# marvinx97/cloud

Measured on AMD Instinct MI355X. Metric: images/sec ResNet-50 via run() at 1/2/4/8 MI355X; run()→first-step latency, higher is better.
Workload: dtype bf16

## Files before the change

cloud_amd/config.py:

```python
from __future__ import annotations

import os
from dataclasses import dataclass


@dataclass(frozen=True)
class Var:
    name: str
    type: type
    default: object
    doc: str
    area: str


_VARS = [
    Var("CLOUD_AMD_JOBS_DIR", str, "./jobs", "where run() stages job directories", "launcher"),
    Var("CLOUD_AMD_HOME", str, "~/.cloud_amd", "per-user state: the job-id index (jobs/<id> -> job directory) that "
        "python -m cloud_amd.jobs uses to find a job from any directory", "launcher"),
    Var("CLOUD_AMD_STAGE_COPY", bool, False, "stage code files by copying too (default: code "
        "hard-linked, every other file copied; a running job then never sees in-place edits of its sources)", "launcher"),
    Var("CLOUD_AMD_CPU_AFFINITY", bool, True, "launcher pins each GPU rank to the cores of its GPU's NUMA node "
        "(KFD io_links + sysfs cpulist), split between the ranks on that node; 0 = leave placement to the OS",
        "launcher"),
    Var("CLOUD_AMD_NUMA_ROOT", str, "/sys/devices/system/node", "sysfs NUMA-node tree read for rank CPU placement "
# ... 28 lines not shown
        "M, N >= 256), 'reg' (register staging); any other name selects 'auto'", "ops"),
    Var("CLOUD_AMD_WGRAD_BLOCKS", int, 512, "convolution weight gradients: split-K so that about this many "
        "workgroups run (tiles x splits); fewer splits = less fp32 slab traffic, more = fuller CUs", "ops"),
    Var("CLOUD_AMD_WGRAD_BLOCKS_SMALLM", int, 512, "convolution weight gradients with <= 128 output channels "
        "(ResNet stem, layers 1-2): split-K workgroup target", "ops"),
    Var("CLOUD_AMD_STEM_WGRAD_BLOCKS", int, 2048, "space-to-depth stem weight gradient (the last kernel of the "
        "backward pass): split-K workgroup target", "ops"),
    Var("CLOUD_AMD_DENSE_WGRAD_BLOCKS", int, 640, "dense-layer weight gradients (BERT): split-K workgroup target "
        "(round 4, same box: 640 -> 6,993 / 6,993 seq/s, 768 -> 6,962 / 6,952, 1024 -> 6,892 / 6,911, 512 -> "
        "6,865 / 6,896; profiles/r4_s36/)",
        "ops"),
    Var("CLOUD_AMD_DENSE_WGRAD_256", bool, False, "dense-layer weight gradients whose 256 x 256 tiles times a split "
        "count fill one round of the chip (BERT QKV / FFN) run on the two-phase 256 core with that split (measured "
        "3 % slower on BERT than the 128 core's 1024-workgroup split: 6,749 / 6,754 vs 6,952 / 6,940 seq/s)", "ops"),
    Var("CLOUD_AMD_TAPMASK", bool, True, "convolutions: tap-mask / incremental buffer-mode gather loaders; 0 keeps "
        "the general per-chunk decode loaders (A/B runs)", "ops"),
    Var("CLOUD_AMD_SPLIT_XCD", bool, True, "split-K GEMM/conv grids: give each XCD contiguous (split, tile) "
        "ranges so the tiles of one K chunk share an L2; 0 remaps tiles only (A/B runs)", "ops"),
    Var("CLOUD_AMD_BN_APPLY_BLOCKS", int, 0, "BatchNorm apply passes (fwd y/mask, bwd dz): total workgroups of "
        "the HBM stream; 0 = the reduction kernels' tiling", "ops"),
    Var("CLOUD_AMD_BN_APPLY_ILV", bool, True, "BatchNorm apply passes: 1 = RP-row groups dealt round-robin to "
        "the workgroups (one contiguous sweep); 0 = one contiguous row chunk per workgroup", "ops"),
    Var("CLOUD_AMD_CONV_TALL", bool, True, "<= 64-channel 3x3 convolutions (fwd, stride-1 dgrad): 256 x 64 tiles "
        "with 4 x 1 waves; 0 = 128 x 64 with 2 x 2 waves", "ops"),
    Var("CLOUD_AMD_STEM_LDS", bool, True, "space-to-depth stem convolution forward on the LDS-resident patch + filter "
        "kernel (csrc/include/ca_conv_stem.h); 0 = the implicit-GEMM row-segment loader", "ops"),
    Var("CLOUD_AMD_STEM_TALL", bool, True, "space-to-depth stem convolution on the tall 256 x 64 tiles too (0.88 -> "
        "0.72 ms per call at b1024); 0 = 128 x 64 tiles (A/B runs)", "ops"),
    Var("CLOUD_AMD_STEM_BWD_RECOMPUTE", bool, True, "ResNet stem tail backward: a statistics-only max-pool "
        "backward pass, then the BN-backward apply recomputes the pooled gradient per 2x2 block (the 112x112 "
        "gradient is never written: 3.3 GB fewer per step at b1024).  With the window loads issued ahead of "
        "any branch: 0.65 + 0.90 ms against 1.09 + 0.94 for write-then-apply, +0.8 % end to end "
        "(profiles/r4_s44/); 0 = write g and run the separate apply pass", "ops"),
    Var("CLOUD_AMD_BN_GROUPS_MAX", int, 512, "BatchNorm statistics: most groups of the first-level reduction of the "
        "per-tile partial rows (1..512; ~64 rows per group)", "ops"),
    Var("CLOUD_AMD_GEMM_LIB", str, "never", "plain bf16 GEMMs (bias / accumulate only, no fused epilogue): 'never' "
        "(default: every GEMM on the in-tree kernels, the same engine on every box and rank), 'auto' (diagnostic: "
        "times the in-tree kernel against hipBLASLt once per shape and keeps the faster), 'always' "
        "(ops/raw.py PlainGemmPolicy)", "ops"),
    Var("CLOUD_AMD_GEMM_PRW", bool, True, "forward 1x1 convolutions with N = 256, K = 64 (ResNet layer-1 conv3 "
        "and shortcut): persistent resident-weight core (csrc/include/ca_gemm_prw.h); 0 = the tiled 128 core",
        "ops"),
    Var("CLOUD_AMD_GEMM_PRWN", bool, True, "forward 1x1 convolutions N = 512 / K = 128 and N = 1024 / K = 256 with "
        "BN statistics (ResNet stage-2 / stage-3 conv3): the persistent core with the weight resident in column "
        "chunks (ca_gemm_prw.h); 0 = the tiled 128 core", "ops"),
    Var("CLOUD_AMD_SMALLK_SET", str, "", "bench/smallk_gemm.py shape set ('conv3': the conv3 expansions of "
        "stages 2-4)", "bench"),
    Var("CLOUD_AMD_EPI_PF", bool, True, "GEMM epilogues that read memory or run an activation (BN-statistics "
        "forward 1x1 convs, BERT bias/GELU/GELU'/beta dense layers): 4 staged output rows in flight per trip", "ops"),
    Var("CLOUD_AMD_ATTN_FUSED_BWD", bool, True, "attention at S = 64 / 128: one workgroup per (batch, head) for "
        "the forward and a single fused backward kernel; 0 keeps the 64-query-block kernels", "ops"),
    Var("CLOUD_AMD_CONV_HALO_WGRAD", bool, True, "the weight gradient of the same 3x3 / 64-channel / width-56 "
        "convolutions on the LDS-resident kernel (ca_conv_halo.h conv3x3_halo_wgrad: 64 x 576 partial in registers, "
        "one fp32 slab per workgroup); 0 = implicit GEMM (A/B)", "ops"),
    Var("CLOUD_AMD_LN_BWD16", bool, False, "LayerNorm backward on 16-wave blocks, one row per wave, the block's "
        "partials summed by a fixed LDS tree (measured 2.8 % slower on BERT beside the weight-gradient side stream; "
        "default: 4-wave blocks walking four rows per wave)", "ops"),
    Var("CLOUD_AMD_GEMM_256X96", bool, True, "forward GEMMs whose 256 x 96 grid fills whole rounds while the 128 x "
        "128 grid leaves a partial one (BERT QKV, M = 8192, N = 2304) run on 256 x 96 tiles; 0 = off (A/B)", "ops"),
    Var("CLOUD_AMD_BN_FIN_RPG", int, 512, "BatchNorm statistics finalize: partial rows per group block (64-512)", "ops"),
    Var("CLOUD_AMD_BN_FIN_MERGED", bool, True, "BatchNorm statistics from many partial rows: group reduction and "
        "per-channel finalize in ONE launch (last block per 64 channels finalizes, agent-scope ticket); 0 = two "
        "launches (A/B runs)", "ops"),
    Var("CLOUD_AMD_CONV_HALO", int, 1, "3x3 / stride-1 / 64-channel convolutions at width 56 (ResNet-50 "
        "stage 1) forward and input gradient on the LDS-resident kernel (ca_conv_halo.h: input patch and all 9 taps "
        "in LDS, persistent grid); 0 = implicit-GEMM tiles, 2 = halo kernel without the software-pipelined "
# ... 198 lines not shown
```

cloud_amd/models/resnet.py:

```python
from __future__ import annotations

import torch
import torch.nn as nn

from . import fused_block
from .. import config
from ..ops import conv as conv_ops
from ..ops import pooling as pool_ops
from .layers import BatchNormAct, Conv2d, GlobalAvgPool, Linear, MaxPool2d


class Bottleneck(nn.Module):
    expansion = 4

    def __init__(self, cin, width, stride=1, dtype=torch.bfloat16, device=None, zero_init_residual=True):
        super().__init__()
        cout = width * self.expansion
        self.conv1 = Conv2d(cin, width, 1, dtype=dtype, device=device)
        self.bn1 = BatchNormAct(width, relu=True, device=device)
        self.conv2 = Conv2d(width, width, 3, stride=stride, padding=1, dtype=dtype, device=device)
        self.bn2 = BatchNormAct(width, relu=True, device=device)
        self.conv3 = Conv2d(width, cout, 1, dtype=dtype, device=device)
        self.bn3 = BatchNormAct(cout, relu=True, zero_init=zero_init_residual, device=device)
        self.fused_stats = True
        self.fused_block = True
        self.downsample = None
        if stride != 1 or cin != cout:
            self.downsample = nn.ModuleDict({
                "conv": Conv2d(cin, cout, 1, stride=stride, dtype=dtype, device=device),
                "bn": BatchNormAct(cout, relu=False, device=device),
            })

    def forward(self, x, next_block=None):
        if self.fused_block and fused_block.can_fuse(self, x):
            return fused_block.bottleneck_forward(self, x, next_block)
        fused_block.check_not_pending(x)
        identity = x
        fs = self.fused_stats
        if self.downsample is not None:
            identity = self.downsample["bn"](self.downsample["conv"](x, stats=fs))
        out = self.bn1(self.conv1(x, stats=fs))
        out = self.bn2(self.conv2(out, stats=fs))
        return self.bn3(self.conv3(out, stats=fs), residual=identity)


class ResNet(nn.Module):
    def __init__(self, layers=(3, 4, 6, 3), num_classes=1000, in_channels=3, stem_channels_pad=0,
                 dtype=torch.bfloat16, device=None, zero_init_residual=True):
        super().__init__()
        self.in_channels = in_channels
        self.stem_cin = in_channels + stem_channels_pad
        self.conv1 = Conv2d(self.stem_cin, 64, 7, stride=2, padding=3, dtype=dtype, device=device)
        self.bn1 = BatchNormAct(64, relu=True, device=device)
        self.maxpool = MaxPool2d(3, 2, 1)
        self.stem_s2d = True
        blocks = []
        cin = 64
        for i, (n, width) in enumerate(zip(layers, (64, 128, 256, 512))):
            for j in range(n):
                stride = 2 if (j == 0 and i > 0) else 1
                blocks.append(Bottleneck(cin, width, stride, dtype=dtype, device=device,
                                         zero_init_residual=zero_init_residual))
                cin = width * Bottleneck.expansion
        self.layers = nn.Sequential(*blocks)
        self.pool = GlobalAvgPool()
        self.fc = Linear(cin, num_classes, dtype=dtype, device=device)

    def forward(self, x):
        c1 = self.conv1
        if self.stem_s2d and x.shape[-1] == self.in_channels and conv_ops.stem_s2d_ok(x, c1.weight, c1.stride,
                                                                                         c1.padding):
            x = self._stem_tail(conv_ops.stem_conv_s2d(x, c1.weight, stats=True))
        else:
            if self.stem_cin != self.in_channels:
                x = torch.nn.functional.pad(x, (0, self.stem_cin - self.in_channels))
            x = self._stem_tail(self.conv1(x, stats=True))
        if self.layers._forward_hooks or self.layers._forward_pre_hooks:
            x = self.layers(x)
        else:
            blocks = list(self.layers)
            for i, blk in enumerate(blocks):
                x = blk(x, blocks[i + 1] if i + 1 < len(blocks) else None)
        return self.fc(self.pool(x))

    def _stem_tail(self, out):
        z, part = out if isinstance(out, tuple) else (out, None)
        if config.get("CLOUD_AMD_STEM_TAIL") and pool_ops.stem_tail_ok(z, self.bn1, self.maxpool, part):
            return pool_ops.stem_bn_relu_maxpool(z, self.bn1, part)
        return self.maxpool(self.bn1((z, part) if part is not None else z))


def resnet50(**kw):
    kw.setdefault("stem_channels_pad", 5)
    return ResNet((3, 4, 6, 3), **kw)


def resnet18_like_small(**kw):
    return ResNet((1, 1, 1, 1), **kw)
```

cloud_amd/ops/conv.py:

```python
from __future__ import annotations

import os

import torch
import torch.nn.functional as F

from .. import config
from . import _ext, gemm, raw


def _out(n, k, s, p):
    return (n + 2 * p - k) // s + 1


def _conv_mode():
    return os.environ.get("CLOUD_AMD_CONV", "native")


def _native_conv_ok(x, w):
    Cin = x.shape[-1]
    Cout = w.shape[0]
    return (x.dtype == torch.bfloat16 and w.dtype == torch.bfloat16 and Cin % 8 == 0 and Cout % 8 == 0
            and x.is_contiguous() and x.numel() < 2 ** 31)

# ... 70 lines not shown
    Cout = g.shape[0]
    return g.view(Cout, 4, 4, 2, 2, 4).permute(0, 1, 3, 2, 4, 5).reshape(Cout, 8, 8, 4)[:, :7, :7, :cx]


class _StemS2DFn(torch.autograd.Function):

    @staticmethod
    def forward(ctx, x, w, param, stats):
        ext = _ext.load(required=True)
        N, H, W, cx = x.shape
        Cout = w.shape[0]
        OH, OW = _out(H, 7, 2, 3), _out(W, 7, 2, 3)
        Hs, Ws = OH + 3, OW + 3
        st = _ext.stream_handle(x.device)
        xs = torch.empty((N, Hs, Ws, 16), dtype=torch.bfloat16, device=x.device)
        ext.stem_s2d(x.data_ptr(), xs.data_ptr(), N, H, W, cx, Hs, Ws, 3, st)
        ws = _s2d_weight(w, cx)
        y = torch.empty((N, OH, OW, Cout), dtype=torch.bfloat16, device=x.device)
        ext.conv_fwd(xs.data_ptr(), ws.data_ptr(), y.data_ptr(), N, Hs, Ws, 16, Cout, 4, 4, 1, 1, 0, 0,
                     _ext.ptr(stats), st)
        ctx.save_for_backward(xs)
        ctx.param, ctx.cx, ctx.wshape = param, cx, w.shape
        return y

    @staticmethod
    def backward(ctx, dy):
        from . import raw

        (xs,) = ctx.saved_tensors
        dy = dy.contiguous()
        Cout = dy.shape[-1]
        g = torch.zeros((Cout, 4, 4, 16), dtype=torch.float32, device=dy.device)
        raw.conv_wgrad(dy, xs, g.shape, 1, 0, out=g, beta=0.0, blocks=config.get("CLOUD_AMD_STEM_WGRAD_BLOCKS"))
        gw = _s2d_weight_grad(g, ctx.cx)
        param = ctx.param
        sink = gemm._grad_sink(param) if param is not None else None
        if sink is not None:
            sink[..., :ctx.cx] += gw.to(sink.dtype)
            from ..parallel import ddp

            ddp.notify_grad_ready(param)
            return None, None, None, None
        full = torch.zeros(ctx.wshape, dtype=torch.float32, device=dy.device)
        full[..., :ctx.cx] = gw
        if param is not None:
            return None, None, full.to(param.dtype), None
        return None, full.to(torch.bfloat16), None, None


def stem_s2d_ok(x, w, stride, padding):
    return (_conv_mode() == "native" and x.is_cuda and x.dtype == torch.bfloat16 and w.dtype == torch.bfloat16
            and tuple(w.shape[1:3]) == (7, 7) and stride == 2 and padding == 3 and x.shape[-1] <= 4
            and x.shape[-1] <= w.shape[-1] and x.is_contiguous() and not x.requires_grad and _ext.use_native(x, w))


def stem_conv_s2d(x, w, stats=False):
    N, H, W, _ = x.shape
    Cout = w.shape[0]
    OH, OW = _out(H, 7, 2, 3), _out(W, 7, 2, 3)
    part = None
    if stats:
        rows = _ext.load(required=True).conv_stat_rows(N, OH + 3, OW + 3, 16, Cout, 4, 4, 1, 1, 0, 0)
        part = torch.empty((rows, 2, Cout), dtype=torch.float32, device=x.device)
    param = w if (w.is_leaf and w.requires_grad) else None
    y = _StemS2DFn.apply(x, w.detach() if param is not None else w, param, part)
    return (y, part) if stats else y


def stats_buffer(rows, channels, device):
    return torch.empty(((rows + 127) // 128, 2, channels), dtype=torch.float32, device=device)


def conv2d_nhwc(x, w, bias=None, stride=1, padding=0, stats=False):
    N, H, W, Cin = x.shape
    Cout, KH, KW, Cin_w = w.shape
    assert Cin == Cin_w, f"channel mismatch {Cin} vs {Cin_w}"
    native = _conv_mode() == "native" and x.is_cuda and _native_conv_ok(x, w) and _ext.use_native(x, w)
    part = None
    if KH == 1 and KW == 1 and padding == 0 and stride == 1:
        x2 = x.reshape(N * H * W, Cin)
# ... 21 lines not shown
```

csrc/bindings.cpp:

```cpp
#include <atomic>
#include <mutex>
#include <hip/hip_runtime.h>
#include <pybind11/pybind11.h>
#include <pybind11/stl.h>
#include <stdint.h>

#include <stdexcept>
#include <string>
#include <vector>

namespace py = pybind11;
typedef uint16_t bf16_t;

extern "C" {
int ca_sgd_step(float*, void*, int, float*, bf16_t*, const float*, const float*, long, int, int, hipStream_t);
int ca_adam_step(float*, void*, int, float*, float*, bf16_t*, const float*, const float*, long, int, int, hipStream_t);
int ca_rmsprop_step(float*, void*, int, float*, float*, bf16_t*, const float*, const float*, long, int, hipStream_t);
int ca_sumsq(const void*, int, long, float*, hipStream_t);
int ca_scale(void*, int, long, const float*, hipStream_t);
long ca_bn_workspace_floats(long, int);
int ca_bn_fwd(const bf16_t*, const bf16_t*, bf16_t*, long, int, const float*, const float*, float, float,
              float*, float*, float*, float*, float*, float*, int, uint8_t*, hipStream_t);
int ca_bn_apply(const bf16_t*, const bf16_t*, bf16_t*, long, int, const float*, int, hipStream_t);
int ca_bn_fwd_partials(const bf16_t*, const bf16_t*, bf16_t*, long, int, const float*, int, const float*, const float*,
// ... 21 lines not shown
                           hipStream_t);
int ca_gemm_xa_dw(const bf16_t*, const bf16_t*, const uint8_t*, const float*, const float*, const float*, long,
                  const bf16_t*, long, bf16_t*, long, int, int, int, float, const bf16_t*, const uint8_t*,
                  const bf16_t*, const uint8_t*, float*, const bf16_t*, float*, const bf16_t*, long, void*, int, float,
                  float*, int, hipStream_t);
int ca_dgrad_gemm(int, const bf16_t*, long, const bf16_t*, long, bf16_t*, long, int, int, int, float, const bf16_t*,
                  const uint8_t*, const bf16_t*, const uint8_t*, float*, hipStream_t, const bf16_t*, float*, int, int,
                  int);
int ca_conv_dgrad_bnstats(const bf16_t*, const bf16_t*, bf16_t*, int, int, int, int, int, int, int, int, int, int,
                          int, float, const bf16_t*, const uint8_t*, float*, hipStream_t);
int ca_u8_normalize(const uint8_t*, bf16_t*, long, int, const float*, const float*, hipStream_t);
int ca_stem_s2d(const bf16_t*, bf16_t*, int, int, int, int, int, int, int, hipStream_t);
int ca_softmax_xent(const void*, int, const int64_t*, int, int, float, float, float*, float*, void*, hipStream_t);
int ca_softmax_xent_batch(const void*, long, int, const int64_t*, int, int, float, float, float*, float*, void*, float*,
                          float,
                          hipStream_t);
int ca_maxpool_fwd(const bf16_t*, bf16_t*, uint8_t*, int, int, int, int, int, int, int, int, int, hipStream_t);
int ca_maxpool_bwd(const bf16_t*, const uint8_t*, bf16_t*, int, int, int, int, int, int, int, int, int, hipStream_t);
int ca_gap_fwd(const bf16_t*, void*, int, int, int, int, hipStream_t);
int ca_gap_bwd(const void*, int, bf16_t*, int, int, int, hipStream_t);
int ca_gmp_fwd(const bf16_t*, bf16_t*, float*, int, int, int, hipStream_t);
int ca_gmp_bwd(const void*, int, const bf16_t*, const bf16_t*, const float*, bf16_t*, int, int, int, hipStream_t);
int ca_gemm_bf16(int, const bf16_t*, long, const bf16_t*, long, bf16_t*, long, int, int, int, float*, float,
                 hipStream_t);
int ca_gemm_set_core(int);
int ca_gemm_set_xa_n256(int);
int ca_gemm_stat_rows(int, int, int, long, long, long);
int ca_bn_relu_maxpool_s2k3(const bf16_t*, const float*, bf16_t*, uint8_t*, int, int, int, int, int, int, hipStream_t);
int ca_maxpool_bnstats_parts(int, int, int, int);
int ca_maxpool_bwd_s2k3_bnstats(const bf16_t*, const bf16_t*, const uint8_t*, const bf16_t*, bf16_t*, float*, int, int,
                                int, int, int, int, hipStream_t);
int ca_maxpool_bwd_s2k3_bnapply(const bf16_t*, const bf16_t*, const uint8_t*, const bf16_t*, const float*, bf16_t*, int,
                                int, int, int, int, int, hipStream_t);
int ca_conv_fwd_ex(const bf16_t*, const bf16_t*, bf16_t*, int, int, int, int, int, int, int, int, int, int, int,
                   const float*, int, hipStream_t);
int ca_conv_fwd(const bf16_t*, const bf16_t*, bf16_t*, int, int, int, int, int, int, int, int, int, int, int, float*,
                hipStream_t);
int ca_conv_dgrad(const bf16_t*, const bf16_t*, bf16_t*, int, int, int, int, int, int, int, int, int, int, int, float,
                  hipStream_t, int);
int ca_conv_wgrad(const bf16_t*, const bf16_t*, void*, int, float, int, int, int, int, int, int, int, int, int, int,
                  int, int, float*, hipStream_t);
int ca_splitk_reduce(const float*, int, long, void*, int, float, hipStream_t);
int ca_grad_finalize_multi(const uint64_t*, const float*, int, hipStream_t);
int ca_cls_head_max_labels();
int ca_cls_head_fwd(const bf16_t*, long, const float*, const float*, float*, int, int, int, float, uint64_t,
                    hipStream_t);
int ca_cls_head_bwd(const float*, const bf16_t*, long, const float*, bf16_t*, float*, float*, int, int, int, float,
                    uint64_t, hipStream_t);
int ca_gemm_splitk(int, const bf16_t*, long, const bf16_t*, long, void*, int, float, int, int, int, int, float*,
                   hipStream_t);
int ca_gemm_splitk_effective(int, int);
int ca_gemm_ex(int, const bf16_t*, long, const bf16_t*, long, bf16_t*, long, int, int, int, float*, float, const float*,
               int, bf16_t*, const bf16_t*, long, hipStream_t);
long ca_ln_workspace_floats(long, int);
int ca_ln_fwd(const bf16_t*, const bf16_t*, const float*, const float*, bf16_t*, bf16_t*, float*, float*, long, int,
              float, float, uint64_t, float, uint64_t, const float*, hipStream_t);
int ca_ln_bwd(const bf16_t*, const bf16_t*, const float*, const float*, const float*, bf16_t*, bf16_t*, float*, float*,
              int, float*, long, int, float, uint64_t, float, uint64_t, hipStream_t, float*);
long ca_colsum_workspace_floats(long, int);
int ca_colsum(const bf16_t*, long, int, long, float*, int, float*, hipStream_t);
int ca_act_grad(const bf16_t*, long, int, const bf16_t*, bf16_t*, long, int, int, hipStream_t);
int ca_pad_cols(const void*, long, int, void*, int, long, long, int, hipStream_t);
int ca_slice_acc(const float*, long, void*, int, long, int, hipStream_t);
int ca_pad_cols_multi(const long*, int, hipStream_t);
int ca_splitk_bias_act(const float*, int, long, int, const float*, int, bf16_t*, hipStream_t);
int ca_embed_sum(const int32_t*, const int32_t*, const float*, const float*, const float*, bf16_t*, long, int, int, int,
// ... 221 lines not shown
  m.def("gemm_bf16", [](int layout, u64 A, long lda, u64 B, long ldb, u64 C, long ldc, int M, int N, int K,
                        u64 stats, float beta, u64 s) {
    check(ca_gemm_bf16(layout, P(const bf16_t*, A), lda, P(const bf16_t*, B), ldb, P(bf16_t*, C), ldc, M, N, K,
                       P(float*, stats), beta, S(s)), "gemm_bf16");
  });
  m.def("conv_fwd", [](u64 x, u64 w, u64 y, int Nb, int H, int W, int Cin, int Cout, int KH, int KW, int sh, int sw,
                       int ph, int pw, u64 stats, u64 s) {
    check(ca_conv_fwd(P(const bf16_t*, x), P(const bf16_t*, w), P(bf16_t*, y), Nb, H, W, Cin, Cout, KH, KW, sh, sw, ph,
                      pw, P(float*, stats), S(s)), "conv_fwd");
  });
  m.def("bn_relu_maxpool_s2k3", [](u64 z, u64 ss, u64 y, u64 idx, int N, int H, int W, int C, int OH, int OW,
                                   u64 s) {
    check(ca_bn_relu_maxpool_s2k3(P(const bf16_t*, z), P(const float*, ss), P(bf16_t*, y), P(uint8_t*, idx), N, H, W,
                                  C, OH, OW, S(s)), "bn_relu_maxpool_s2k3");
  });
  m.def("gemm_set_core", [](int kind) { return ca_gemm_set_core(kind); });
  m.def("gemm_set_xa_n256", [](int mode) { return ca_gemm_set_xa_n256(mode); });
  m.def("experimental_built", []() { return false; });
  m.def("gemm_set_streamk", [](int) { return -1; });
  m.def("maxpool_bnstats_parts", [](int N, int H, int W, int C) { return ca_maxpool_bnstats_parts(N, H, W, C); });
  m.def("maxpool_bwd_s2k3_bnstats", [](u64 dy, u64 yp, u64 idx, u64 z, u64 g, u64 part, int N, int H, int W, int C,
                                       int OH, int OW, u64 s) {
    check(ca_maxpool_bwd_s2k3_bnstats(P(const bf16_t*, dy), P(const bf16_t*, yp), P(const uint8_t*, idx),
                                      P(const bf16_t*, z), P(bf16_t*, g), P(float*, part), N, H, W, C, OH, OW, S(s)),
          "maxpool_bwd_s2k3_bnstats");
  });
  m.def("maxpool_bwd_s2k3_bnapply", [](u64 dy, u64 yp, u64 idx, u64 z, u64 coef, u64 dz, int N, int H, int W, int C,
                                       int OH, int OW, u64 s) {
    check(ca_maxpool_bwd_s2k3_bnapply(P(const bf16_t*, dy), P(const bf16_t*, yp), P(const uint8_t*, idx),
                                      P(const bf16_t*, z), P(const float*, coef), P(bf16_t*, dz), N, H, W, C, OH, OW,
                                      S(s)),
          "maxpool_bwd_s2k3_bnapply");
  });
  m.def("conv_fwd_ex", [](u64 x, u64 w, u64 y, int Nb, int H, int W, int Cin, int Cout, int KH, int KW, int sh,
                          int sw, int ph, int pw, u64 bias, int act, u64 s) {
    check(ca_conv_fwd_ex(P(const bf16_t*, x), P(const bf16_t*, w), P(bf16_t*, y), Nb, H, W, Cin, Cout, KH, KW, sh, sw,
                         ph, pw, P(const float*, bias), act, S(s)), "conv_fwd_ex");
  });
  m.def("conv_dgrad", [](u64 dy, u64 w, u64 dx, int Nb, int H, int W, int Cin, int Cout, int KH, int KW, int sh,
                         int sw, int ph, int pw, float beta, u64 s, int skip_empty) {
    check(ca_conv_dgrad(P(const bf16_t*, dy), P(const bf16_t*, w), P(bf16_t*, dx), Nb, H, W, Cin, Cout, KH, KW, sh, sw,
                        ph, pw, beta, S(s), skip_empty), "conv_dgrad");
  }, py::arg("dy"), py::arg("w"), py::arg("dx"), py::arg("Nb"), py::arg("H"), py::arg("W"), py::arg("Cin"),
        py::arg("Cout"), py::arg("KH"), py::arg("KW"), py::arg("sh"), py::arg("sw"), py::arg("ph"), py::arg("pw"),
        py::arg("beta"), py::arg("s"), py::arg("skip_empty") = 0);
  m.def("conv_wgrad", [](u64 dy, u64 x, u64 dw, int dw_bf16, float beta, int Nb, int H, int W, int Cin, int Cout,
                         int KH, int KW, int sh, int sw, int ph, int pw, int splits, u64 ws, u64 s) {
    check(ca_conv_wgrad(P(const bf16_t*, dy), P(const bf16_t*, x), P(void*, dw), dw_bf16, beta, Nb, H, W, Cin, Cout,
                        KH, KW, sh, sw, ph, pw, splits, P(float*, ws), S(s)), "conv_wgrad");
  });
  m.def("grad_finalize_multi", [](const std::vector<uint64_t>& jobs, const std::vector<float>& betas, u64 s) {
    const int n = (int)betas.size();
    if ((long)jobs.size() != 12L * n) throw std::runtime_error("grad_finalize_multi: 12 fields per job");
    check(ca_grad_finalize_multi(jobs.data(), betas.data(), n, S(s)), "grad_finalize_multi");
  });
  m.def("cls_head_max_labels", []() { return ca_cls_head_max_labels(); });
  m.def("cls_head_fwd", [](u64 pooled, long ldp, u64 wc, u64 bc, u64 logits, int B, int C, int L, float p, u64 seed,
                           u64 s) {
    check(ca_cls_head_fwd(P(const bf16_t*, pooled), ldp, P(const float*, wc), P(const float*, bc), P(float*, logits),
                          B, C, L, p, seed, S(s)), "cls_head_fwd");
  });
  m.def("cls_head_bwd", [](u64 dl, u64 pooled, long ldp, u64 wc, u64 dpre, u64 gwc, u64 gbc, int B, int C, int L,
                           float p, u64 seed, u64 s) {
    check(ca_cls_head_bwd(P(const float*, dl), P(const bf16_t*, pooled), ldp, P(const float*, wc), P(bf16_t*, dpre),
                          P(float*, gwc), P(float*, gbc), B, C, L, p, seed, S(s)), "cls_head_bwd");
  });
// ... 96 lines not shown
```

csrc/kernels/pool.hip:

```cpp
#include "ca_common.h"

namespace {

__global__ void __launch_bounds__(256) maxpool_fwd_kernel(const bf16_t* __restrict__ x, bf16_t* __restrict__ y,
                                                         uint8_t* __restrict__ idx, int N, int H, int W, int C,
                                                         int OH, int OW, int k, int s, int p) {
  const int CT = C / 8;
  const long total = (long)N * OH * OW * CT;
  for (long t = (long)blockIdx.x * blockDim.x + threadIdx.x; t < total; t += (long)gridDim.x * blockDim.x) {
    const int vc = (int)(t % CT);
    long r = t / CT;
    const int ow = (int)(r % OW); r /= OW;
    const int oh = (int)(r % OH);
    const int n = (int)(r / OH);
    float best[8];
    uint8_t bi[8];
#pragma unroll
    for (int j = 0; j < 8; ++j) { best[j] = -INFINITY; bi[j] = 0; }
    for (int kh = 0; kh < k; ++kh) {
      const int h = oh * s - p + kh;
      if (h < 0 || h >= H) continue;
      for (int kw = 0; kw < k; ++kw) {
        const int w = ow * s - p + kw;
        if (w < 0 || w >= W) continue;
        us8 v = *reinterpret_cast<const us8*>(x + (((long)n * H + h) * W + w) * C + vc * 8);
#pragma unroll
        for (int j = 0; j < 8; ++j) {
          float f = bf2f(v[j]);
          if (f > best[j]) { best[j] = f; bi[j] = (uint8_t)(kh * k + kw); }
        }
      }
    }
    us8 o;
// ... 475 lines not shown
    const int vc = (int)(t % (uint32_t)CT);
    uint32_t r = t / (uint32_t)CT;
    const int bj = (int)(r % (uint32_t)Wb); r /= (uint32_t)Wb;
    const int bi = (int)(r % (uint32_t)Hb);
    const int n = (int)(r / (uint32_t)Hb);
    float A[8], B[8], D[8];
#pragma unroll
    for (int j = 0; j < 8; ++j) {
      A[j] = coef[vc * 8 + j];
      B[j] = coef[C + vc * 8 + j];
      D[j] = coef[2 * C + vc * 8 + j];
    }
    float acc[2][2][8];
    stem_block_grad(dy, ypool, idx, n, bi, bj, vc, C, OH, OW, acc);
#pragma unroll
    for (int a = 0; a < 2; ++a) {
      const int h = 2 * bi + a;
      if (h >= H) continue;
#pragma unroll
      for (int b = 0; b < 2; ++b) {
        const int w = 2 * bj + b;
        if (w >= W) continue;
        const long off = (long)((n * H + h) * W) * C + (w * C + vc * 8);
        const us8 zv = *reinterpret_cast<const us8*>(z + off);
        us8 o;
#pragma unroll
        for (int j = 0; j < 8; ++j) o[j] = f2bf(bn_bwd_affine(A[j], acc[a][b][j], B[j], bf2f(zv[j]), D[j]));
        *reinterpret_cast<us8*>(dz + off) = o;
      }
    }
  }
}

extern "C" {

int ca_bn_relu_maxpool_s2k3(const bf16_t* z, const float* ss, bf16_t* y, uint8_t* idx, int N, int H, int W, int C,
                            int OH, int OW, hipStream_t st) {
  if (C % 8 != 0 || OH != (H - 1) / 2 + 1 || OW != (W - 1) / 2 + 1) return -1;
  const long total = (long)N * OH * ((OW + 1) / 2) * (C / 8);
  if (total >= (1L << 31) || (long)N * H * W >= (1L << 31)) return -1;
  const int grid = (int)((total + 255) / 256 < 65536 ? (total + 255) / 256 : 65536);
  bn_relu_maxpool_s2k3_kernel<<<grid, 256, 0, st>>>(z, ss, y, idx, N, H, W, C, OH, OW);
  CA_LAUNCH_CHECK();
  return 0;
}

int ca_maxpool_bnstats_parts(int N, int H, int W, int C) {
  const long total = (long)N * ((H + 1) / 2) * ((W + 1) / 2) * (C / 8);
  const long b = (total + 255) / 256;
  return (int)(b < 1024 ? b : 1024);
}

int ca_maxpool_bwd_s2k3_bnstats(const bf16_t* dy, const bf16_t* ypool, const uint8_t* idx, const bf16_t* z, bf16_t* g,
                                float* part, int N, int H, int W, int C, int OH, int OW, hipStream_t st) {
  if (C % 8 != 0 || 256 % (C / 8) != 0 || OH != (H - 1) / 2 + 1 || OW != (W - 1) / 2 + 1) return -1;
  if ((long)N * ((H + 1) / 2) * ((W + 1) / 2) * (C / 8) >= (1L << 31) || (long)N * H * W >= (1L << 31))
    return -1;
  const int grid = ca_maxpool_bnstats_parts(N, H, W, C);
  if (g) maxpool_bwd_s2k3_bnstats_kernel<true><<<grid, 256, 0, st>>>(dy, ypool, idx, z, g, part, N, H, W, C, OH, OW);
  else maxpool_bwd_s2k3_bnstats_kernel<false><<<grid, 256, 0, st>>>(dy, ypool, idx, z, g, part, N, H, W, C, OH, OW);
  CA_LAUNCH_CHECK();
  return 0;
}

int ca_maxpool_bwd_s2k3_bnapply(const bf16_t* dy, const bf16_t* ypool, const uint8_t* idx, const bf16_t* z,
                                const float* coef, bf16_t* dz, int N, int H, int W, int C, int OH, int OW,
                                hipStream_t st) {
  if (C % 8 != 0 || OH != (H - 1) / 2 + 1 || OW != (W - 1) / 2 + 1) return -1;
  const long total = (long)N * ((H + 1) / 2) * ((W + 1) / 2) * (C / 8);
  if (total >= (1L << 31) || (long)N * H * W >= (1L << 31)) return -1;
  maxpool_bwd_s2k3_bnapply_kernel<<<ca_stream_grid(total, 256), 256, 0, st>>>(dy, ypool, idx, z, coef, dz, N, H, W,
                                                                              C, OH, OW);
  CA_LAUNCH_CHECK();
  return 0;
}


int ca_stem_s2d(const bf16_t* x, bf16_t* y, int N, int H, int W, int C, int Hs, int Ws, int pad, hipStream_t st) {
  if (C < 1 || C > 4) return -1;
  const long total = (long)N * Hs * Ws;
  stem_s2d_kernel<<<(unsigned)((total + 255) / 256), 256, 0, st>>>(x, y, N, H, W, C, Hs, Ws, pad);
  CA_LAUNCH_CHECK();
  return 0;
}

int ca_maxpool_fwd(const bf16_t* x, bf16_t* y, uint8_t* idx, int N, int H, int W, int C, int OH, int OW,
                   int k, int s, int p, hipStream_t st) {
  if (C % 8 || k * k > 255) return -1;
  const long total = (long)N * OH * OW * (C / 8);
  maxpool_fwd_kernel<<<ca_stream_grid(total, 256), 256, 0, st>>>(x, y, idx, N, H, W, C, OH, OW, k, s, p);
  CA_LAUNCH_CHECK();
  return 0;
}

int ca_maxpool_bwd(const bf16_t* dy, const uint8_t* idx, bf16_t* dx, int N, int H, int W, int C, int OH, int OW,
                   int k, int s, int p, hipStream_t st) {
  if (C % 8) return -1;
  const long total = (long)N * H * W * (C / 8);
  if (k == 3 && s == 2 && p == 1 && OH == (H - 1) / 2 + 1 && OW == (W - 1) / 2 + 1) {
    const long blocks = (long)N * ((H + 1) / 2) * ((W + 1) / 2) * (C / 8);
    maxpool_bwd_s2k3_kernel<<<ca_stream_grid(blocks, 256), 256, 0, st>>>(dy, idx, dx, N, H, W, C, OH, OW);
    CA_LAUNCH_CHECK();
    return 0;
  }
  maxpool_bwd_kernel<<<ca_stream_grid(total, 256), 256, 0, st>>>(dy, idx, dx, N, H, W, C, OH, OW, k, s, p);
  CA_LAUNCH_CHECK();
  return 0;
}

// ... 40 lines not shown
```

Measured before the change: 16120.

## Fuse stem weight gradient into BN-backward apply pass via LDS-resident dz

Adds a fused autograd node for the ResNet stem (conv + BN + ReLU + maxpool). In backward, the BN apply pass writes dz into LDS and feeds it directly to MFMAs against the space-to-depth input patch, producing per-block weight-gradient partials that a split-K reduce then sums. This avoids writing the 112x112x64 dz to HBM and reading it back in a separate wgrad kernel. The cost is a persistent kernel with more LDS and a partial-sum reduction, and it only applies to specific stem shapes.

After: 16260 (median of 6 runs). No clear change (+0.9%).

```diff
diff --git a/cloud_amd/config.py b/cloud_amd/config.py
--- a/cloud_amd/config.py
+++ b/cloud_amd/config.py
@@ -84,6 +84,11 @@
         "gradient is never written: 3.3 GB fewer per step at b1024).  With the window loads issued ahead of "
         "any branch: 0.65 + 0.90 ms against 1.09 + 0.94 for write-then-apply, +0.8 % end to end "
         "(profiles/r4_s44/); 0 = write g and run the separate apply pass", "ops"),
+    Var("CLOUD_AMD_STEM_WGRAD_FUSED", bool, True, "ResNet stem backward: the stem weight gradient is computed inside "
+        "the BN-backward apply pass (csrc/include/ca_conv_stem_wgrad.h: dz goes to LDS and into the MFMAs, never to "
+        "memory; one autograd node for stem convolution + tail, ops/stem.py).  Needs the space-to-depth LDS stem "
+        "shapes (output width 112, height a multiple of 4), CLOUD_AMD_STEM_TAIL and "
+        "CLOUD_AMD_STEM_BWD_RECOMPUTE; 0 = apply pass writes dz, split-K weight gradient reads it back", "ops"),
     Var("CLOUD_AMD_BN_GROUPS_MAX", int, 512, "BatchNorm statistics: most groups of the first-level reduction of the "
         "per-tile partial rows (1..512; ~64 rows per group)", "ops"),
     Var("CLOUD_AMD_GEMM_LIB", str, "never", "plain bf16 GEMMs (bias / accumulate only, no fused epilogue): 'never' "
diff --git a/cloud_amd/models/resnet.py b/cloud_amd/models/resnet.py
--- a/cloud_amd/models/resnet.py
+++ b/cloud_amd/models/resnet.py
@@ -7,6 +7,7 @@
 from .. import config
 from ..ops import conv as conv_ops
 from ..ops import pooling as pool_ops
+from ..ops import stem as stem_ops
 from .layers import BatchNormAct, Conv2d, GlobalAvgPool, Linear, MaxPool2d
 
 
@@ -70,7 +71,10 @@
         c1 = self.conv1
         if self.stem_s2d and x.shape[-1] == self.in_channels and conv_ops.stem_s2d_ok(x, c1.weight, c1.stride,
                                                                                          c1.padding):
-            x = self._stem_tail(conv_ops.stem_conv_s2d(x, c1.weight, stats=True))
+            if stem_ops.stem_fused_ok(x, c1.weight, self.bn1, self.maxpool):
+                x = stem_ops.stem_fused(x, c1.weight, self.bn1)
+            else:
+                x = self._stem_tail(conv_ops.stem_conv_s2d(x, c1.weight, stats=True))
         else:
             if self.stem_cin != self.in_channels:
                 x = torch.nn.functional.pad(x, (0, self.stem_cin - self.in_channels))
diff --git a/cloud_amd/ops/conv.py b/cloud_amd/ops/conv.py
--- a/cloud_amd/ops/conv.py
+++ b/cloud_amd/ops/conv.py
@@ -126,20 +126,24 @@
         Cout = dy.shape[-1]
         g = torch.zeros((Cout, 4, 4, 16), dtype=torch.float32, device=dy.device)
         raw.conv_wgrad(dy, xs, g.shape, 1, 0, out=g, beta=0.0, blocks=config.get("CLOUD_AMD_STEM_WGRAD_BLOCKS"))
-        gw = _s2d_weight_grad(g, ctx.cx)
-        param = ctx.param
-        sink = gemm._grad_sink(param) if param is not None else None
-        if sink is not None:
-            sink[..., :ctx.cx] += gw.to(sink.dtype)
-            from ..parallel import ddp
+        dw, dparam = _stem_weight_grad_out(g, ctx.cx, ctx.param, ctx.wshape)
+        return None, dw, dparam, None
 
-            ddp.notify_grad_ready(param)
-            return None, None, None, None
-        full = torch.zeros(ctx.wshape, dtype=torch.float32, device=dy.device)
-        full[..., :ctx.cx] = gw
-        if param is not None:
-            return None, None, full.to(param.dtype), None
-        return None, full.to(torch.bfloat16), None, None
+
+def _stem_weight_grad_out(g, cx, param, wshape):
+    gw = _s2d_weight_grad(g, cx)
+    sink = gemm._grad_sink(param) if param is not None else None
+    if sink is not None:
+        sink[..., :cx] += gw.to(sink.dtype)
+        from ..parallel import ddp
+
+        ddp.notify_grad_ready(param)
+        return None, None
+    full = torch.zeros(wshape, dtype=torch.float32, device=g.device)
+    full[..., :cx] = gw
+    if param is not None:
+        return None, full.to(param.dtype)
+    return full.to(torch.bfloat16), None
 
 
 def stem_s2d_ok(x, w, stride, padding):
diff --git a/cloud_amd/ops/stem.py b/cloud_amd/ops/stem.py
--- /dev/null
+++ b/cloud_amd/ops/stem.py
@@ -0,0 +1,88 @@
+from __future__ import annotations
+
+import torch
+
+from .. import config
+from . import _ext, conv, raw
+
+
+def _out(n, k, s, p):
+    return (n + 2 * p - k) // s + 1
+
+
+class _StemFusedFn(torch.autograd.Function):
+    @staticmethod
+    def forward(ctx, x, w, param, gamma, beta, running_mean, running_var, eps, momentum):
+        ext = _ext.load(required=True)
+        N, H, W, cx = x.shape
+        C = w.shape[0]
+        OH, OW = _out(H, 7, 2, 3), _out(W, 7, 2, 3)
+        Hs, Ws = OH + 3, OW + 3
+        PH, PW = (OH - 1) // 2 + 1, (OW - 1) // 2 + 1
+        st = _ext.stream_handle(x.device)
+        xs = torch.empty((N, Hs, Ws, 16), dtype=torch.bfloat16, device=x.device)
+        ext.stem_s2d(x.data_ptr(), xs.data_ptr(), N, H, W, cx, Hs, Ws, 3, st)
+        ws = conv._s2d_weight(w, cx)
+        rows = ext.conv_stat_rows(N, Hs, Ws, 16, C, 4, 4, 1, 1, 0, 0)
+        part = torch.empty((rows, 2, C), dtype=torch.float32, device=x.device)
+        z = torch.empty((N, OH, OW, C), dtype=torch.bfloat16, device=x.device)
+        ext.conv_fwd(xs.data_ptr(), ws.data_ptr(), z.data_ptr(), N, Hs, Ws, 16, C, 4, 4, 1, 1, 0, 0,
+                     part.data_ptr(), st)
+        stats = raw.bn_fwd_stats(z, gamma, beta, running_mean, running_var, eps, momentum, part)
+        y = torch.empty((N, PH, PW, C), dtype=torch.bfloat16, device=x.device)
+        idx = torch.empty((N, PH, PW, C), dtype=torch.uint8, device=x.device)
+        ext.bn_relu_maxpool_s2k3(z.data_ptr(), stats[2 * C:].data_ptr(), y.data_ptr(), idx.data_ptr(), N, OH, OW, C,
+                                 PH, PW, st)
+        ctx.save_for_backward(xs, z, stats, y, idx, gamma)
+        ctx.has_beta = beta is not None
+        ctx.param, ctx.cx, ctx.wshape = param, cx, w.shape
+        return y
+
+    @staticmethod
+    def backward(ctx, dy):
+        ext = _ext.load(required=True)
+        xs, z, stats, y, idx, gamma = ctx.saved_tensors
+        N, OH, OW, C = z.shape
+        PH, PW = y.shape[1], y.shape[2]
+        dev = z.device
+        dy = dy.contiguous()
+        st = _ext.stream_handle(dev)
+        parts = torch.empty((ext.maxpool_bnstats_parts(N, OH, OW, C), 2, C), dtype=torch.float32, device=dev)
+        dgamma = torch.empty(C, dtype=torch.float32, device=dev) if gamma is not None else None
+        dbeta = torch.empty(C, dtype=torch.float32, device=dev) if ctx.has_beta else None
+        ext.maxpool_bwd_s2k3_bnstats(dy.data_ptr(), y.data_ptr(), idx.data_ptr(), z.data_ptr(), 0, parts.data_ptr(),
+                                     N, OH, OW, C, PH, PW, st)
+        coef = raw.bn_bwd_coef(C, N * OH * OW, gamma, stats, parts, dgamma=dgamma, dbeta=dbeta)
+        g = stem_wgrad_fused(dy, y, idx, z, coef, xs)
+        dw, dparam = conv._stem_weight_grad_out(g, ctx.cx, ctx.param, ctx.wshape)
+        return None, dw, dparam, dgamma, dbeta, None, None, None, None
+
+
+def stem_wgrad_fused(dy, y, idx, z, coef, xs, blocks=0, dz_out=None, return_partials=False):
+    ext = _ext.load(required=True)
+    N, OH, OW, C = z.shape
+    nparts = ext.stem_wgrad_fused_parts(N, OH, blocks)
+    assert nparts > 0 and OW == 112 and C == 64 and xs.shape == (N, OH + 3, OW + 3, 16), "not a fused-stem shape"
+    st = _ext.stream_handle(z.device)
+    ws = torch.empty((nparts, C, 4, 4, 16), dtype=torch.float32, device=z.device)
+    ext.stem_wgrad_fused(dy.data_ptr(), y.data_ptr(), idx.data_ptr(), z.data_ptr(), coef.data_ptr(), xs.data_ptr(),
+                         ws.data_ptr(), N, OH, blocks, _ext.ptr(dz_out), st)
+    g = torch.empty((C, 4, 4, 16), dtype=torch.float32, device=z.device)
+    ext.splitk_reduce(ws.data_ptr(), nparts, C * 256, g.data_ptr(), 0, 0.0, st)
+    return (g, ws) if return_partials else g
+
+
+def stem_fused_ok(x, w, bn, pool):
+    if not (config.get("CLOUD_AMD_STEM_WGRAD_FUSED") and config.get("CLOUD_AMD_STEM_TAIL")
+            and config.get("CLOUD_AMD_STEM_BWD_RECOMPUTE") and config.get("CLOUD_AMD_STEM_LDS")):
+        return False
+    N, H, W, _ = x.shape
+    OH, OW = _out(H, 7, 2, 3), _out(W, 7, 2, 3)
+    return (bn.training and bn.relu and (pool.k, pool.stride, pool.padding) == (3, 2, 1) and w.shape[0] == 64
+            and OW == 112 and OH % 4 == 0 and _ext.load(required=True).stem_wgrad_fused_parts(N, OH, 0) > 0)
+
+
+def stem_fused(x, w, bn):
+    param = w if (w.is_leaf and w.requires_grad) else None
+    return _StemFusedFn.apply(x, w.detach() if param is not None else w, param, bn.weight, bn.bias,
+                              bn.running_mean, bn.running_var, bn.eps, bn.momentum)
diff --git a/csrc/bindings.cpp b/csrc/bindings.cpp
--- a/csrc/bindings.cpp
+++ b/csrc/bindings.cpp
@@ -77,6 +77,9 @@
                                 int, int, int, int, hipStream_t);
 int ca_maxpool_bwd_s2k3_bnapply(const bf16_t*, const bf16_t*, const uint8_t*, const bf16_t*, const float*, bf16_t*, int,
                                 int, int, int, int, int, hipStream_t);
+int ca_stem_wgrad_fused_parts(int, int, int);
+int ca_stem_wgrad_fused(const bf16_t*, const bf16_t*, const uint8_t*, const bf16_t*, const float*, const bf16_t*, float*,
+                        int, int, int, bf16_t*, hipStream_t);
 int ca_conv_fwd_ex(const bf16_t*, const bf16_t*, bf16_t*, int, int, int, int, int, int, int, int, int, int, int,
                    const float*, int, hipStream_t);
 int ca_conv_fwd(const bf16_t*, const bf16_t*, bf16_t*, int, int, int, int, int, int, int, int, int, int, int, float*,
@@ -364,6 +367,14 @@
                                       S(s)),
           "maxpool_bwd_s2k3_bnapply");
   });
+  m.def("stem_wgrad_fused_parts", [](int N, int OH, int blocks) { return ca_stem_wgrad_fused_parts(N, OH, blocks); });
+  m.def("stem_wgrad_fused", [](u64 dy, u64 yp, u64 idx, u64 z, u64 coef, u64 xs, u64 ws, int N, int OH, int blocks,
+                               u64 dz, u64 s) {
+    check(ca_stem_wgrad_fused(P(const bf16_t*, dy), P(const bf16_t*, yp), P(const uint8_t*, idx), P(const bf16_t*, z),
+                              P(const float*, coef), P(const bf16_t*, xs), P(float*, ws), N, OH, blocks,
+                              P(bf16_t*, dz), S(s)),
+          "stem_wgrad_fused");
+  });
   m.def("conv_fwd_ex", [](u64 x, u64 w, u64 y, int Nb, int H, int W, int Cin, int Cout, int KH, int KW, int sh,
                           int sw, int ph, int pw, u64 bias, int act, u64 s) {
     check(ca_conv_fwd_ex(P(const bf16_t*, x), P(const bf16_t*, w), P(bf16_t*, y), Nb, H, W, Cin, Cout, KH, KW, sh, sw,
diff --git a/csrc/include/ca_conv_stem_wgrad.h b/csrc/include/ca_conv_stem_wgrad.h
--- /dev/null
+++ b/csrc/include/ca_conv_stem_wgrad.h
@@ -0,0 +1,139 @@
+#pragma once
+#include "ca_conv_stem.h"
+
+namespace ca {
+
+struct StemWgParams {
+  const bf16_t* dy;
+  const bf16_t* ypool;
+  const uint8_t* idx;
+  const bf16_t* z;
+  const float* coef;
+  const bf16_t* xs;
+  float* ws;
+  bf16_t* dz;
+  int N, OH;
+};
+
+constexpr int SWG_TR = 2, SWG_WAVES = 4, SWG_NT = SWG_WAVES * 64;
+constexpr int SWG_TP = SWG_TR * STEM_OW;
+constexpr int SWG_PR = SWG_TR + 3;
+constexpr int SWG_PCH = SWG_PR * STEM_PW * 2;
+constexpr int SWG_PPT = (SWG_PCH + SWG_NT - 1) / SWG_NT;
+constexpr int SWG_ITEMS = (SWG_TR / 2) * (STEM_OW / 2) * (STEM_C / 8);
+constexpr int SWG_ROUNDS = (SWG_ITEMS + SWG_NT - 1) / SWG_NT;
+constexpr int SWG_PIMG = SWG_PR * STEM_PW * STEM_CI;
+
+template <bool WRITE_DZ, class BlockGrad>
+__device__ __forceinline__ void stem_wgrad_fused(const StemWgParams& P, BlockGrad block_grad) {
+  constexpr int C = STEM_C, OW = STEM_OW, PW = STEM_PW, NT = SWG_NT, TP = SWG_TP;
+  __shared__ __attribute__((aligned(256))) short smem[TP * C + SWG_PIMG];
+  short* dimg = smem;
+  short* pimg = smem + TP * C;
+  __shared__ float cimg[3 * C];
+
+  const int tid = threadIdx.x, lane = tid & 63, wave = tid >> 6;
+  const int OH = P.OH, rgroups = OH / SWG_TR, ntiles = P.N * rgroups;
+  const long img = (long)(OH + 3) * PW * STEM_CI;
+  const int vc = tid & 7;
+
+  f4v acc[4][4];
+#pragma unroll
+  for (int i = 0; i < 4; ++i)
+#pragma unroll
+    for (int j = 0; j < 4; ++j) acc[i][j] = f4v{0.f, 0.f, 0.f, 0.f};
+  if (tid < 3 * C) cimg[tid] = P.coef[tid];
+
+  const int fq = (lane & 15) >> 2, fp = lane & 3, fg = lane >> 4;
+  const short* abase[4];
+#pragma unroll
+  for (int i = 0; i < 4; ++i)
+    abase[i] = dimg + (8 * fg + fq) * C + (((2 * i + (fp >> 1)) ^ nc_swz<64>(8 * fg + fq)) << 3) + 4 * (fp & 1);
+  const short* bbase = pimg + (wave * PW + 8 * fg + fq) * STEM_CI + 4 * fp;
+  const short* bbase3 = bbase + (fg >= 2 ? 3 * STEM_CI : 0);
+  auto tr8 = [](const short* lo_p, const short* hi_p) {
+    s4v lo = __builtin_amdgcn_ds_read_tr16_b64_v4i16((lds_s4v*)(lo_p));
+    s4v hi = __builtin_amdgcn_ds_read_tr16_b64_v4i16((lds_s4v*)(hi_p));
+    s8v v = {lo[0], lo[1], lo[2], lo[3], hi[0], hi[1], hi[2], hi[3]};
+    return __builtin_bit_cast(bf16x8, v);
+  };
+  auto frag_load = [&](int ks, bf16x8 (&af)[4], bf16x8 (&bfr)[4]) {
+#pragma unroll
+    for (int i = 0; i < 4; ++i) af[i] = tr8(abase[i] + ks * 32 * C, abase[i] + (ks * 32 + 4) * C);
+    const short* bb = (ks == 3 ? bbase3 : bbase) + (32 * ks + (ks >= 4 ? 3 : 0)) * STEM_CI;
+#pragma unroll
+    for (int j = 0; j < 4; ++j) bfr[j] = tr8(bb + j * STEM_CI, bb + (j + 4) * STEM_CI);
+  };
+
+  for (int t = blockIdx.x; t < ntiles; t += gridDim.x) {
+    const int n = t / rgroups, bi = t % rgroups;
+    s8v pv[SWG_PPT];
+    const bf16_t* psrc = P.xs + n * img + (long)bi * SWG_TR * PW * STEM_CI;
+#pragma unroll
+    for (int i = 0; i < SWG_PPT; ++i) {
+      const int e = tid + i * NT;
+      pv[i] = *reinterpret_cast<const s8v*>(psrc + (e < SWG_PCH ? e : SWG_PCH - 1) * 8);
+    }
+    __syncthreads();
+#pragma unroll
+    for (int i = 0; i < SWG_PPT; ++i) {
+      const int e = tid + i * NT;
+      if (e < SWG_PCH) *reinterpret_cast<s8v*>(pimg + e * 8) = pv[i];
+    }
+#pragma unroll
+    for (int rd = 0; rd < SWG_ROUNDS; ++rd) {
+      const int it = tid + rd * NT;
+      if (it < SWG_ITEMS) {
+        const int bj = it >> 3;
+        const long zoff = (((long)n * OH + 2 * bi) * OW + 2 * bj) * C + vc * 8;
+        us8 zvs[2][2];
+#pragma unroll
+        for (int a = 0; a < 2; ++a)
+#pragma unroll
+          for (int b = 0; b < 2; ++b) zvs[a][b] = *reinterpret_cast<const us8*>(P.z + zoff + (long)(a * OW + b) * C);
+        float g[2][2][8];
+        block_grad(n, bi, bj, vc, g);
+        float A[8], B[8], D[8];
+#pragma unroll
+        for (int j = 0; j < 8; ++j) {
+          A[j] = cimg[vc * 8 + j];
+          B[j] = cimg[C + vc * 8 + j];
+          D[j] = cimg[2 * C + vc * 8 + j];
+        }
+#pragma unroll
+        for (int a = 0; a < 2; ++a)
+#pragma unroll
+          for (int b = 0; b < 2; ++b) {
+            us8 o;
+#pragma unroll
+            for (int j = 0; j < 8; ++j) o[j] = f2bf(bn_bwd_affine(A[j], g[a][b][j], B[j], bf2f(zvs[a][b][j]), D[j]));
+            const int k = a * OW + 2 * bj + b;
+            *reinterpret_cast<us8*>(dimg + k * C + ((vc ^ nc_swz<64>(k)) << 3)) = o;
+            if constexpr (WRITE_DZ) *reinterpret_cast<us8*>(P.dz + zoff + (long)(a * OW + b) * C) = o;
+          }
+      }
+    }
+    __syncthreads();
+    bf16x8 fa[2][4], fb[2][4];
+    frag_load(0, fa[0], fb[0]);
+#pragma unroll
+    for (int ks = 0; ks < TP / 32; ++ks) {
+      if (ks + 1 < TP / 32) frag_load(ks + 1, fa[(ks + 1) & 1], fb[(ks + 1) & 1]);
+      __builtin_amdgcn_sched_barrier(0);
+#pragma unroll
+      for (int j = 0; j < 4; ++j)
+#pragma unroll
+        for (int i = 0; i < 4; ++i)
+          acc[i][j] = __builtin_amdgcn_mfma_f32_16x16x32_bf16(fb[ks & 1][j], fa[ks & 1][i], acc[i][j], 0, 0, 0);
+      __builtin_amdgcn_sched_barrier(0);
+    }
+  }
+  float* dst = P.ws + (long)blockIdx.x * C * 256;
+#pragma unroll
+  for (int i = 0; i < 4; ++i)
+#pragma unroll
+    for (int j = 0; j < 4; ++j)
+      *reinterpret_cast<f4v*>(dst + (i * 16 + (lane & 15)) * 256 + (wave * 4 + j) * 16 + 4 * (lane >> 4)) = acc[i][j];
+}
+
+}
diff --git a/csrc/kernels/pool.hip b/csrc/kernels/pool.hip
--- a/csrc/kernels/pool.hip
+++ b/csrc/kernels/pool.hip
@@ -1,4 +1,5 @@
 #include "ca_common.h"
+#include "ca_conv_stem_wgrad.h"
 
 namespace {
 
@@ -540,6 +541,13 @@
   }
 }
 
+template <bool WRITE_DZ>
+__global__ void __launch_bounds__(ca::SWG_NT) stem_wgrad_fused_kernel(ca::StemWgParams P) {
+  ca::stem_wgrad_fused<WRITE_DZ>(P, [&](int n, int bi, int bj, int vc, float (&g)[2][2][8]) {
+    stem_block_grad(P.dy, P.ypool, P.idx, n, bi, bj, vc, ca::STEM_C, P.OH / 2, ca::STEM_OW / 2, g);
+  });
+}
+
 extern "C" {
 
 int ca_bn_relu_maxpool_s2k3(const bf16_t* z, const float* ss, bf16_t* y, uint8_t* idx, int N, int H, int W, int C,
@@ -583,6 +591,41 @@
   return 0;
 }
 
+
+int ca_stem_wgrad_fused_parts(int N, int OH, int blocks) {
+  if (N < 1 || OH < 4 || OH % ca::STEM_TR != 0) return -1;
+  const long tiles = (long)N * (OH / ca::SWG_TR);
+  if ((long)N * (OH / 2) * (ca::STEM_OW / 2) * (ca::STEM_C / 8) >= (1L << 31) ||
+      (long)N * OH * ca::STEM_OW >= (1L << 31))
+    return -1;
+  long g = blocks;
+  if (blocks <= 0) {
+    static int slots = 0;
+    if (!slots) {
+      int dev = 0, per_cu = 0;
+      hipDeviceProp_t prop;
+      const bool ok = hipGetDevice(&dev) == hipSuccess && hipGetDeviceProperties(&prop, dev) == hipSuccess &&
+                      prop.multiProcessorCount > 0 &&
+                      hipOccupancyMaxActiveBlocksPerMultiprocessor(&per_cu, stem_wgrad_fused_kernel<false>, ca::SWG_NT,
+                                                                   0) == hipSuccess &&
+                      per_cu > 0;
+      slots = ok ? prop.multiProcessorCount * per_cu : 512;
+    }
+    g = slots;
+  }
+  return (int)(g < tiles ? g : tiles);
+}
+
+int ca_stem_wgrad_fused(const bf16_t* dy, const bf16_t* ypool, const uint8_t* idx, const bf16_t* z, const float* coef,
+                        const bf16_t* xs, float* ws, int N, int OH, int blocks, bf16_t* dz_out, hipStream_t st) {
+  const int g = ca_stem_wgrad_fused_parts(N, OH, blocks);
+  if (g < 1) return -1;
+  ca::StemWgParams P{dy, ypool, idx, z, coef, xs, ws, dz_out, N, OH};
+  if (dz_out) stem_wgrad_fused_kernel<true><<<g, ca::SWG_NT, 0, st>>>(P);
+  else stem_wgrad_fused_kernel<false><<<g, ca::SWG_NT, 0, st>>>(P);
+  CA_LAUNCH_CHECK();
+  return 0;
+}
 
 int ca_stem_s2d(const bf16_t* x, bf16_t* y, int N, int H, int W, int C, int Hs, int Ws, int pad, hipStream_t st) {
   if (C < 1 || C > 4) return -1;
```
